# cloneofsimo/paint-with-words-sd

Measured on NVIDIA H100. Metric: unet_steps_per_sec_512sq_cfg, higher is better.
Workload: dtype f16

## Files before the change

### paint_with_words_sd_b200/csrc/pww_abi.cu

```cuda
#include <stdio.h>
#include <string.h>

#include "pww_common.cuh"
#include "xattn_tc.cuh"
#include "xattn_fused2.cuh"
#include "attn_tc.cuh"
#include "unet_ops.cuh"
#include "sampler_step.cuh"
#include "control_inject.cuh"
#include <stdlib.h>

namespace {

thread_local char g_last_cuda_error[640] = "";

int cuda_fail(cudaError_t e);

bool aligned16(const void* p) { return (reinterpret_cast<uintptr_t>(p) & 15u) == 0; }

bool supported_head_dim(int D) { return D == 40 || D == 64 || D == 80 || D == 160; }

int check_common(const void* q, const void* k, int B, int H, int N, int T, int D, int64_t q_bs, int64_t q_rs,
                 int64_t k_bs, int64_t k_rs) {
  if (!q || !k || B <= 0 || H <= 0 || N <= 0 || T <= 0 || D <= 0) return PWW_ERR_BAD_ARG;
  if (!aligned16(q) || !aligned16(k)) return PWW_ERR_BAD_ARG;
  if ((q_bs | q_rs | k_bs | k_rs) & 7) return PWW_ERR_BAD_ARG;
  if (q_rs < (int64_t)H * D || k_rs < (int64_t)H * D) return PWW_ERR_BAD_ARG;
  if (!supported_head_dim(D) || !pww::core::supported_keys(T)) return PWW_ERR_UNSUPPORTED;
  return PWW_OK;
}

template <int D_, int KC_>
struct Shape {
  static constexpr int D = D_, KC = KC_;
};
template <int D, typename F>
cudaError_t with_chunks(int T, F&& f) {
  switch (pww::core::chunks_of(T)) {
    case 1: return f(Shape<D, 1>{});
    case 2: return f(Shape<D, 2>{});
    case 3: return f(Shape<D, 3>{});
  }
  return cudaErrorInvalidValue;
}
template <typename F>
cudaError_t with_shape(int D, int T, F&& f) {
  switch (D) {
    case 40: return with_chunks<40>(T, f);
    case 64: return with_chunks<64>(T, f);
    case 80: return with_chunks<80>(T, f);
    case 160: return with_chunks<160>(T, f);
  }
  return cudaErrorInvalidValue;
}

size_t align_up(size_t x, size_t a) { return (x + a - 1) / a * a; }

int stats_slots_per_image(int, int) { return 2048; }

int cuda_fail(cudaError_t e) {
  snprintf(g_last_cuda_error, sizeof(g_last_cuda_error), "%s: %s %s", cudaGetErrorName(e), cudaGetErrorString(e),
           pww::tc::tc_error_buf());
  pww::tc::tc_error_buf()[0] = 0;
  return PWW_ERR_CUDA;
}

}

extern "C" {

int pww_version(void) { return 300; }

const char* pww_status_str(int status) {
  switch (status) {
    case PWW_OK: return "ok";
    case PWW_ERR_BAD_ARG: return "bad argument (null/misaligned pointer, non-positive size or stride not a multiple of 8)";
    case PWW_ERR_UNSUPPORTED: return "unsupported shape or dtype (head dim must be 40/64/80/160, T <= 80, 154 or 231)";
    case PWW_ERR_CUDA: return "CUDA error (see pww_last_cuda_error)";
    case PWW_ERR_WORKSPACE: return "workspace too small (see pww_xattn_workspace_bytes)";
    default: return "unknown status";
  }
}

const char* pww_last_cuda_error(void) { return g_last_cuda_error; }

int pww_device_supported(void) {
  int dev = 0, major = 0;
  cudaError_t e = cudaGetDevice(&dev);
  if (e != cudaSuccess) return cuda_fail(e);
  e = cudaDeviceGetAttribute(&major, cudaDevAttrComputeCapabilityMajor, dev);
  if (e != cudaSuccess) return cuda_fail(e);
  return major == 9 ? 1 : 0;
}

size_t pww_xattn_workspace_bytes(int B, int H, int N, int T, int D) {
  (void)T; (void)D;
  if (B <= 0 || H <= 0 || N <= 0) return 0;
  return align_up((size_t)B * sizeof(unsigned int), 256) +
         (size_t)B * stats_slots_per_image(H, N) * sizeof(pww::StatPartial);
}

}

namespace {

template <typename E>
int xattn_stats(const void* q, const void* k, int B, int H, int N, int T, int D, int64_t q_batch_stride,
                int64_t q_row_stride, int64_t k_batch_stride, int64_t k_row_stride, int stat, const int32_t* kinds,
                bool per_image, const int32_t* wmap_index, float* stats, void* workspace, size_t workspace_bytes,
                void* stream) {
  int rc = check_common(q, k, B, H, N, T, D, q_batch_stride, q_row_stride, k_batch_stride, k_row_stride);
  if (rc) return rc;
  if (!stats || !workspace) return PWW_ERR_BAD_ARG;
  if (per_image ? !kinds : (stat != PWW_STAT_MAX && stat != PWW_STAT_STD)) return PWW_ERR_BAD_ARG;
  if (workspace_bytes < pww_xattn_workspace_bytes(B, H, N, T, D)) return PWW_ERR_WORKSPACE;
  pww::XattnParams<E> p;
  memset(&p, 0, sizeof(p));
  p.q = (const E*)q; p.k = (const E*)k;
  p.B = B; p.H = H; p.N = N; p.T = T; p.D = D;
  p.q_bs = q_batch_stride; p.q_rs = q_row_stride; p.k_bs = k_batch_stride; p.k_rs = k_row_stride;
  p.wmap_index = wmap_index; p.stat = stat; p.stat_kind = per_image ? kinds : nullptr; p.stats_out = stats;
  p.counters = (unsigned int*)workspace;
  p.partials = (pww::StatPartial*)((char*)workspace + align_up((size_t)B * sizeof(unsigned int), 256));
  cudaStream_t s = (cudaStream_t)stream;
  {
    if (pww::tc::stats_slots() > stats_slots_per_image(H, N)) return PWW_ERR_WORKSPACE;
    for (int b0 = 0; b0 < B; b0 += pww::tc::kMaxBatch) {
      pww::XattnParams<E> c = p;
      c.B = (B - b0) < pww::tc::kMaxBatch ? (B - b0) : pww::tc::kMaxBatch;
      c.q = p.q + (int64_t)b0 * p.q_bs;
      c.k = p.k + (int64_t)b0 * p.k_bs;
      c.wmap_index = p.wmap_index ? p.wmap_index + b0 : nullptr;
      c.stat_kind = p.stat_kind ? p.stat_kind + b0 : nullptr;
      c.stats_out = p.stats_out + b0;
      const cudaError_t e = with_shape(D, T, [&](auto k) { return pww::tc::launch_stats<k.D, k.KC>(c, s); });
      if (e != cudaSuccess) return cuda_fail(e);
    }
    return PWW_OK;
  }
}

template <typename E>
int xattn_fwd(const void* q, const void* k, const void* v, void* out, int B, int H, int N, int T, int D,
              int64_t q_batch_stride, int64_t q_row_stride, int64_t k_batch_stride, int64_t k_row_stride,
              int64_t o_batch_stride, int64_t o_row_stride, const float* wmap, int64_t wmap_batch_stride,
              const int32_t* wmap_index, const float* stats, const float* g_sigma, int64_t g_stride, float scale,
              void* stream) {
  int rc = check_common(q, k, B, H, N, T, D, q_batch_stride, q_row_stride, k_batch_stride, k_row_stride);
  if (rc) return rc;
  if (!v || !out || !aligned16(v) || !aligned16(out)) return PWW_ERR_BAD_ARG;
  if ((o_batch_stride | o_row_stride) & 7 || o_row_stride < (int64_t)H * D) return PWW_ERR_BAD_ARG;
  if (wmap && (!stats || !g_sigma)) return PWW_ERR_BAD_ARG;
  pww::XattnParams<E> p;
  memset(&p, 0, sizeof(p));
  p.q = (const E*)q; p.k = (const E*)k; p.v = (const E*)v; p.out = (E*)out;
  p.B = B; p.H = H; p.N = N; p.T = T; p.D = D;
  p.q_bs = q_batch_stride; p.q_rs = q_row_stride; p.k_bs = k_batch_stride; p.k_rs = k_row_stride;
  p.o_bs = o_batch_stride; p.o_rs = o_row_stride;
  p.wmap = wmap; p.wmap_bs = wmap_batch_stride; p.wmap_index = wmap_index;
  p.stats = stats; p.g_sigma = g_sigma; p.g_stride = g_stride; p.scale = scale;
  cudaStream_t s = (cudaStream_t)stream;
  {
    for (int b0 = 0; b0 < B; b0 += pww::tc::kMaxBatch) {
      pww::XattnParams<E> c = p;
      c.B = (B - b0) < pww::tc::kMaxBatch ? (B - b0) : pww::tc::kMaxBatch;
      c.q = p.q + (int64_t)b0 * p.q_bs;
      c.k = p.k + (int64_t)b0 * p.k_bs;
      c.v = p.v + (int64_t)b0 * p.k_bs;
      c.out = p.out + (int64_t)b0 * p.o_bs;
      c.wmap_index = (p.wmap && p.wmap_index) ? p.wmap_index + b0 : nullptr;
      c.stats = p.stats ? p.stats + b0 : nullptr;
      c.g_sigma = p.g_sigma ? p.g_sigma + (int64_t)b0 * p.g_stride : nullptr;
      if (p.wmap && !p.wmap_index) c.wmap = p.wmap + (int64_t)b0 * p.wmap_bs;
      const cudaError_t e = with_shape(D, T, [&](auto k) { return pww::tc::launch_fwd<k.D, k.KC>(c, s); });
      if (e != cudaSuccess) return cuda_fail(e);
    }
    return PWW_OK;
  }
}

template <typename E>
int xattn_fused(const void* q, const void* k, const void* v, void* out, int B, int H, int N, int T, int D,
                int64_t q_batch_stride, int64_t q_row_stride, int64_t k_batch_stride, int64_t k_row_stride,
                int64_t o_batch_stride, int64_t o_row_stride, const void* mpack, int64_t mpack_batch_stride, int Bw,
                const int8_t* cidx, const int32_t* wmap_index, int stat, const int32_t* kinds, bool per_image,
                const float* g_sigma, float scale, float* stats, void* workspace, size_t workspace_bytes,
                void* stream) {
  int rc = check_common(q, k, B, H, N, T, D, q_batch_stride, q_row_stride, k_batch_stride, k_row_stride);
  if (rc) return rc;
  if (!v || !out || !aligned16(v) || !aligned16(out)) return PWW_ERR_BAD_ARG;
  if ((o_batch_stride | o_row_stride) & 7 || o_row_stride < (int64_t)H * D || o_batch_stride <= 0) return PWW_ERR_BAD_ARG;
  if (mpack) {
    if (!cidx || !g_sigma || !workspace || Bw <= 0 || !aligned16(mpack)) return PWW_ERR_BAD_ARG;
    if ((mpack_batch_stride & 7) || mpack_batch_stride < (int64_t)N * pww::fx::kMW) return PWW_ERR_BAD_ARG;
    if (per_image ? !kinds : (stat != PWW_STAT_MAX && stat != PWW_STAT_STD)) return PWW_ERR_BAD_ARG;
    if (workspace_bytes < pww_xattn_fused_workspace_bytes()) return PWW_ERR_WORKSPACE;
  }
  pww::XattnParams<E> p;
  memset(&p, 0, sizeof(p));
  p.q = (const E*)q; p.k = (const E*)k; p.v = (const E*)v; p.out = (E*)out;
  p.B = B; p.H = H; p.N = N; p.T = T; p.D = D;
  p.q_bs = q_batch_stride; p.q_rs = q_row_stride; p.k_bs = k_batch_stride; p.k_rs = k_row_stride;
  p.o_bs = o_batch_stride; p.o_rs = o_row_stride;
  p.g_sigma = g_sigma; p.g_stride = per_image ? 1 : 0; p.scale = scale; p.stat = stat;
  p.stat_kind = per_image ? kinds : nullptr;
  p.counters = (unsigned int*)workspace;
  p.partials = workspace ? (pww::StatPartial*)((char*)workspace + 512) : nullptr;
  cudaStream_t s = (cudaStream_t)stream;
  int chunk = pww::fx::kMaxBatch;
  {
    const int tiles = pww::ceil_div(N, pww::core::kBM);
    const int hg = pww::ceil_div(H, D == 40 ? pww::fx::Cfg2<40>::G : (D == 64 ? pww::fx::Cfg2<64>::G : 1));
    while (chunk > 1) {
      const int cb = B < chunk ? B : chunk;
      if (pww::fx::fused2_fits(cb, hg, tiles, pww::fx::fused_grid(cb * hg * tiles))) break;
      chunk >>= 1;
    }
  }
  for (int b0 = 0; b0 < B; b0 += chunk) {
    pww::XattnParams<E> c = p;
    c.B = (B - b0) < chunk ? (B - b0) : chunk;
    c.q = p.q + (int64_t)b0 * p.q_bs;
    c.k = p.k + (int64_t)b0 * p.k_bs;
    c.v = p.v + (int64_t)b0 * p.k_bs;
    c.out = p.out + (int64_t)b0 * p.o_bs;
    c.stats_out = stats ? stats + b0 : nullptr;
    c.stat_kind = p.stat_kind ? p.stat_kind + b0 : nullptr;
    c.g_sigma = p.g_sigma ? p.g_sigma + (int64_t)b0 * p.g_stride : nullptr;
    const void* mp = mpack;
    const int8_t* ci = cidx;
    if (mpack && wmap_index) {
      c.wmap_index = wmap_index + b0;
    } else if (mpack) {
      c.wmap_index = nullptr;
      mp = (const __half*)mpack + (int64_t)b0 * mpack_batch_stride;
      ci = cidx + (int64_t)b0 * pww::core::kTP * pww::core::chunks_of(T);
    }
    c.wmap = mpack ? (const float*)mp : nullptr;
    const cudaError_t e =
        with_shape(D, T, [&](auto k) { return pww::fx::launch_fused2<k.D, k.KC>(c, mp, mpack_batch_stride, ci, s); });
    if (e == cudaErrorInvalidConfiguration) return PWW_ERR_UNSUPPORTED;
    if (e != cudaSuccess) return cuda_fail(e);
  }
  return PWW_OK;
}

template <typename E>
int groupnorm_nhwc(const void* x, const void* add, int64_t add_batch_stride, const void* gamma, const void* beta, void* y,
                   int B, int HW, int C, int G, float eps, int silu, void* workspace, size_t workspace_bytes,
                   void* stream) {
  if (!x || !gamma || !beta || !y || !workspace || B <= 0 || HW <= 0 || C <= 0 || G <= 0) return PWW_ERR_BAD_ARG;
  if (!aligned16(x) || !aligned16(y) || !aligned16(gamma) || !aligned16(beta) || (add && !aligned16(add)))
    return PWW_ERR_BAD_ARG;
  if ((C & 7) || (C % G) || G > 64 || (C >> 3) > 1024) return PWW_ERR_UNSUPPORTED;
  if (add && ((add_batch_stride & 7) || add_batch_stride < C)) return PWW_ERR_BAD_ARG;
  if (workspace_bytes < pww_groupnorm_workspace_bytes(B, HW, G)) return PWW_ERR_WORKSPACE;
  pww::uops::GnParams<E> p;
  p.x = (const E*)x; p.add = (const E*)add; p.add_bs = add_batch_stride; p.gamma = (const E*)gamma; p.beta = (const E*)beta;
  p.y = (E*)y;
  char* w = (char*)workspace;
  p.counters = (unsigned int*)w;
  w += align_up((size_t)B * sizeof(unsigned int), 256);
  p.stats = (float*)w;
  w += align_up((size_t)B * G * 2 * sizeof(float), 256);
  p.partial = (float*)w;
  p.B = B; p.HW = HW; p.C = C; p.G = G; p.eps = eps; p.silu = silu;
  p.chunks = pww::uops::gn_chunks(HW);
  p.rows_per_chunk = (HW + p.chunks - 1) / p.chunks;
  cudaStream_t s = (cudaStream_t)stream;
  const int nvec = C >> 3;
  const int rpp = nvec >= 256 ? 1 : 256 / nvec;
  const size_t smem1 = (size_t)rpp * C * 2 * sizeof(float);
  if (smem1 > 48 * 1024) return PWW_ERR_UNSUPPORTED;
  pww::uops::gn_stats_kernel<E><<<dim3(p.chunks, B), nvec * rpp, smem1, s>>>(p);
  int rows_per_block = (int)(((long long)HW * B + 2 * pww::tc::num_sms() - 1) / (2 * pww::tc::num_sms()));
  if (rows_per_block < rpp) rows_per_block = rpp;
  if (rows_per_block > 32) rows_per_block = 32;
  pww::uops::gn_apply_kernel<E><<<dim3((HW + rows_per_block - 1) / rows_per_block, B), nvec * rpp, 0, s>>>(p, rows_per_block);
  cudaError_t e = cudaGetLastError();
  return e == cudaSuccess ? PWW_OK : cuda_fail(e);
}

template <typename E>
int geglu(const void* in, void* out, int64_t M, int I, void* stream) {
  if (!in || !out || M <= 0 || I <= 0 || !aligned16(in) || !aligned16(out)) return PWW_ERR_BAD_ARG;
  if (I & 7) return PWW_ERR_UNSUPPORTED;
  const long long total = (long long)M * (I >> 3);
  long long blocks = (total + 255) / 256;
  const long long cap = (long long)pww::tc::num_sms() * 16;
  if (blocks > cap) blocks = cap;
  pww::uops::geglu_kernel<E><<<(int)blocks, 256, 0, (cudaStream_t)stream>>>((const E*)in, (E*)out, M, I);
  cudaError_t e = cudaGetLastError();
  return e == cudaSuccess ? PWW_OK : cuda_fail(e);
}

template <typename E>
int add_layernorm(const void* x, const void* res, const void* gamma, const void* beta, void* sum_out, void* y, int64_t M,
                  int C, float eps, void* stream) {
  if (!x || !gamma || !beta || !y || M <= 0 || C <= 0) return PWW_ERR_BAD_ARG;
  if (!aligned16(x) || !aligned16(y) || !aligned16(gamma) || !aligned16(beta) || (res && !aligned16(res)) ||
      (sum_out && !aligned16(sum_out)))
    return PWW_ERR_BAD_ARG;
  if ((C & 7) || C > 2048) return PWW_ERR_UNSUPPORTED;
  const int vpl = ((C >> 3) + 31) / 32;
  const int warps = 8;
  const unsigned grid = (unsigned)((M + warps - 1) / warps);
  cudaStream_t s = (cudaStream_t)stream;
  const E *xp = (const E*)x, *rp = (const E*)res, *gp = (const E*)gamma, *bp = (const E*)beta;
  E *sp = (E*)sum_out, *yp = (E*)y;
  switch (vpl) {
    case 1: pww::uops::add_layernorm_kernel<E, 1><<<grid, warps * 32, 0, s>>>(xp, rp, gp, bp, sp, yp, M, C, eps); break;
    case 2: pww::uops::add_layernorm_kernel<E, 2><<<grid, warps * 32, 0, s>>>(xp, rp, gp, bp, sp, yp, M, C, eps); break;
    case 3: pww::uops::add_layernorm_kernel<E, 3><<<grid, warps * 32, 0, s>>>(xp, rp, gp, bp, sp, yp, M, C, eps); break;
    case 4: pww::uops::add_layernorm_kernel<E, 4><<<grid, warps * 32, 0, s>>>(xp, rp, gp, bp, sp, yp, M, C, eps); break;
    case 5: pww::uops::add_layernorm_kernel<E, 5><<<grid, warps * 32, 0, s>>>(xp, rp, gp, bp, sp, yp, M, C, eps); break;
    case 6: pww::uops::add_layernorm_kernel<E, 6><<<grid, warps * 32, 0, s>>>(xp, rp, gp, bp, sp, yp, M, C, eps); break;
    case 7: pww::uops::add_layernorm_kernel<E, 7><<<grid, warps * 32, 0, s>>>(xp, rp, gp, bp, sp, yp, M, C, eps); break;
    case 8: pww::uops::add_layernorm_kernel<E, 8><<<grid, warps * 32, 0, s>>>(xp, rp, gp, bp, sp, yp, M, C, eps); break;
    default: return PWW_ERR_UNSUPPORTED;
  }
  cudaError_t e = cudaGetLastError();
  return e == cudaSuccess ? PWW_OK : cuda_fail(e);
}

template <typename E>
int attn_fwd(const void* q, const void* k, const void* v, void* out, int B, int H, int N, int D, int64_t qkv_batch_stride,
             int64_t qkv_row_stride, int64_t o_batch_stride, int64_t o_row_stride, float scale, void* stream) {
  if (!q || !k || !v || !out || B <= 0 || H <= 0 || N <= 0 || D <= 0) return PWW_ERR_BAD_ARG;
  if (!aligned16(q) || !aligned16(k) || !aligned16(v) || !aligned16(out)) return PWW_ERR_BAD_ARG;
  if ((qkv_batch_stride | qkv_row_stride | o_batch_stride | o_row_stride) & 7) return PWW_ERR_BAD_ARG;
  if (qkv_row_stride < (int64_t)H * D || o_row_stride < (int64_t)H * D) return PWW_ERR_BAD_ARG;
  if (!supported_head_dim(D)) return PWW_ERR_UNSUPPORTED;
  cudaStream_t s = (cudaStream_t)stream;
  cudaError_t e = cudaErrorInvalidValue;
  const int64_t bs = qkv_batch_stride, rs = qkv_row_stride, obs = o_batch_stride, ors = o_row_stride;
  switch (D) {
    case 40: e = pww::fa::launch<40, E>(q, k, v, out, B, H, N, bs, rs, obs, ors, scale, s); break;
    case 64: e = pww::fa::launch<64, E>(q, k, v, out, B, H, N, bs, rs, obs, ors, scale, s); break;
    case 80: e = pww::fa::launch<80, E>(q, k, v, out, B, H, N, bs, rs, obs, ors, scale, s); break;
    case 160: e = pww::fa::launch<160, E>(q, k, v, out, B, H, N, bs, rs, obs, ors, scale, s); break;
  }
  return e == cudaSuccess ? PWW_OK : cuda_fail(e);
}

template <typename E>
int control_inject(int n, void* const* dst, const void* const* res, const int64_t* elems_per_image, int rows,
                   const float* scales, void* stream) {
  if (n < 1 || n > pww::ctl::kMaxLevels || rows < 1 || !dst || !res || !elems_per_image) return PWW_ERR_BAD_ARG;
  pww::ctl::InjectArgs a;
  a.off[0] = 0;
  for (int k = 0; k < n; ++k) {
    const int64_t e = elems_per_image[k];
    if (e <= 0 || (e % pww::ctl::kVec) != 0) return PWW_ERR_BAD_ARG;
    if (!dst[k] || !res[k] || !aligned16(dst[k]) || !aligned16(res[k])) return PWW_ERR_BAD_ARG;
    a.dst[k] = dst[k];
    a.res[k] = res[k];
    a.vec_per_image[k] = e / pww::ctl::kVec;
    a.off[k + 1] = a.off[k] + (int64_t)rows * a.vec_per_image[k];
  }
  for (int k = n; k < pww::ctl::kMaxLevels; ++k) {
    a.dst[k] = nullptr;
    a.res[k] = nullptr;
    a.vec_per_image[k] = 0;
    a.off[k + 1] = a.off[n];
  }
  a.scales = scales;
  a.n = n;
  a.rows = rows;
  const cudaError_t e = pww::ctl::launch_inject<E>(a, (int64_t)pww::tc::num_sms() * 8, (cudaStream_t)stream);
  return e == cudaSuccess ? PWW_OK : cuda_fail(e);
}

}

extern "C" {

int pww_xattn_stats_f16(const void* q, const void* k, int B, int H, int N, int T, int D, int64_t q_batch_stride,
    int64_t q_row_stride, int64_t k_batch_stride, int64_t k_row_stride, int stat, const int32_t* wmap_index,
    float* stats, void* workspace, size_t workspace_bytes, void* stream) {
  return xattn_stats<__half>(
      q, k, B, H, N, T, D, q_batch_stride, q_row_stride, k_batch_stride, k_row_stride, stat, nullptr, false,
      wmap_index, stats, workspace, workspace_bytes, stream);
}
int pww_xattn_stats_bf16(const void* q, const void* k, int B, int H, int N, int T, int D, int64_t q_batch_stride,
    int64_t q_row_stride, int64_t k_batch_stride, int64_t k_row_stride, int stat, const int32_t* wmap_index,
    float* stats, void* workspace, size_t workspace_bytes, void* stream) {
  return xattn_stats<__nv_bfloat16>(
      q, k, B, H, N, T, D, q_batch_stride, q_row_stride, k_batch_stride, k_row_stride, stat, nullptr, false,
      wmap_index, stats, workspace, workspace_bytes, stream);
}

int pww_xattn_stats_multi_f16(const void* q, const void* k, int B, int H, int N, int T, int D, int64_t q_batch_stride,
    int64_t q_row_stride, int64_t k_batch_stride, int64_t k_row_stride, const int32_t* stat, const int32_t* wmap_index,
    float* stats, void* workspace, size_t workspace_bytes, void* stream) {
  return xattn_stats<__half>(
      q, k, B, H, N, T, D, q_batch_stride, q_row_stride, k_batch_stride, k_row_stride, PWW_STAT_MAX, stat, true,
      wmap_index, stats, workspace, workspace_bytes, stream);
}
int pww_xattn_stats_multi_bf16(const void* q, const void* k, int B, int H, int N, int T, int D, int64_t q_batch_stride,
    int64_t q_row_stride, int64_t k_batch_stride, int64_t k_row_stride, const int32_t* stat, const int32_t* wmap_index,
    float* stats, void* workspace, size_t workspace_bytes, void* stream) {
  return xattn_stats<__nv_bfloat16>(
      q, k, B, H, N, T, D, q_batch_stride, q_row_stride, k_batch_stride, k_row_stride, PWW_STAT_MAX, stat, true,
      wmap_index, stats, workspace, workspace_bytes, stream);
}

int pww_xattn_fwd_f16(const void* q, const void* k, const void* v, void* out, int B, int H, int N, int T, int D,
    int64_t q_batch_stride, int64_t q_row_stride, int64_t k_batch_stride, int64_t k_row_stride, int64_t o_batch_stride,
    int64_t o_row_stride, const float* wmap, int64_t wmap_batch_stride, const int32_t* wmap_index, const float* stats,
    const float* g_sigma, float scale, void* stream) {
  return xattn_fwd<__half>(q, k, v, out, B, H, N, T, D, q_batch_stride, q_row_stride, k_batch_stride, k_row_stride,
      o_batch_stride, o_row_stride, wmap, wmap_batch_stride, wmap_index, stats, g_sigma, 0, scale, stream);
}
int pww_xattn_fwd_bf16(const void* q, const void* k, const void* v, void* out, int B, int H, int N, int T, int D,
    int64_t q_batch_stride, int64_t q_row_stride, int64_t k_batch_stride, int64_t k_row_stride, int64_t o_batch_stride,
    int64_t o_row_stride, const float* wmap, int64_t wmap_batch_stride, const int32_t* wmap_index, const float* stats,
    const float* g_sigma, float scale, void* stream) {
  return xattn_fwd<__nv_bfloat16>(
      q, k, v, out, B, H, N, T, D, q_batch_stride, q_row_stride, k_batch_stride, k_row_stride,
      o_batch_stride, o_row_stride, wmap, wmap_batch_stride, wmap_index, stats, g_sigma, 0, scale, stream);
}

int pww_xattn_fwd_multi_f16(const void* q, const void* k, const void* v, void* out, int B, int H, int N, int T, int D,
    int64_t q_batch_stride, int64_t q_row_stride, int64_t k_batch_stride, int64_t k_row_stride, int64_t o_batch_stride,
    int64_t o_row_stride, const float* wmap, int64_t wmap_batch_stride, const int32_t* wmap_index, const float* stats,
    const float* g_sigma, float scale, void* stream) {
  return xattn_fwd<__half>(q, k, v, out, B, H, N, T, D, q_batch_stride, q_row_stride, k_batch_stride, k_row_stride,
      o_batch_stride, o_row_stride, wmap, wmap_batch_stride, wmap_index, stats, g_sigma, 1, scale, stream);
}
int pww_xattn_fwd_multi_bf16(const void* q, const void* k, const void* v, void* out, int B, int H, int N, int T, int D,
    int64_t q_batch_stride, int64_t q_row_stride, int64_t k_batch_stride, int64_t k_row_stride, int64_t o_batch_stride,
    int64_t o_row_stride, const float* wmap, int64_t wmap_batch_stride, const int32_t* wmap_index, const float* stats,
    const float* g_sigma, float scale, void* stream) {
  return xattn_fwd<__nv_bfloat16>(
      q, k, v, out, B, H, N, T, D, q_batch_stride, q_row_stride, k_batch_stride, k_row_stride,
      o_batch_stride, o_row_stride, wmap, wmap_batch_stride, wmap_index, stats, g_sigma, 1, scale, stream);
}

size_t pww_xattn_fused_workspace_bytes(void) { return pww::fx::fused_workspace_bytes(); }

int pww_xattn_fused_f16(const void* q, const void* k, const void* v, void* out, int B, int H, int N, int T, int D,
    int64_t q_batch_stride, int64_t q_row_stride, int64_t k_batch_stride, int64_t k_row_stride, int64_t o_batch_stride,
    int64_t o_row_stride, const void* mpack, int64_t mpack_batch_stride, int Bw, const int8_t* cidx,
    const int32_t* wmap_index, int stat, const float* g_sigma, float scale, float* stats, void* workspace,
    size_t workspace_bytes, void* stream) {
  return xattn_fused<__half>(q, k, v, out, B, H, N, T, D, q_batch_stride, q_row_stride, k_batch_stride, k_row_stride,
      o_batch_stride, o_row_stride, mpack, mpack_batch_stride, Bw, cidx, wmap_index, stat, nullptr, false,
      g_sigma, scale, stats, workspace, workspace_bytes, stream);
}
int pww_xattn_fused_bf16(const void* q, const void* k, const void* v, void* out, int B, int H, int N, int T, int D,
    int64_t q_batch_stride, int64_t q_row_stride, int64_t k_batch_stride, int64_t k_row_stride, int64_t o_batch_stride,
    int64_t o_row_stride, const void* mpack, int64_t mpack_batch_stride, int Bw, const int8_t* cidx,
    const int32_t* wmap_index, int stat, const float* g_sigma, float scale, float* stats, void* workspace,
    size_t workspace_bytes, void* stream) {
  return xattn_fused<__nv_bfloat16>(
      q, k, v, out, B, H, N, T, D, q_batch_stride, q_row_stride, k_batch_stride, k_row_stride,
      o_batch_stride, o_row_stride, mpack, mpack_batch_stride, Bw, cidx, wmap_index, stat, nullptr, false,
      g_sigma, scale, stats, workspace, workspace_bytes, stream);
}

int pww_xattn_fused_multi_f16(const void* q, const void* k, const void* v, void* out, int B, int H, int N, int T, int D,
    int64_t q_batch_stride, int64_t q_row_stride, int64_t k_batch_stride, int64_t k_row_stride, int64_t o_batch_stride,
    int64_t o_row_stride, const void* mpack, int64_t mpack_batch_stride, int Bw, const int8_t* cidx,
    const int32_t* wmap_index, const int32_t* stat, const float* g_sigma, float scale, float* stats, void* workspace,
    size_t workspace_bytes, void* stream) {
  return xattn_fused<__half>(q, k, v, out, B, H, N, T, D, q_batch_stride, q_row_stride, k_batch_stride, k_row_stride,
      o_batch_stride, o_row_stride, mpack, mpack_batch_stride, Bw, cidx, wmap_index, PWW_STAT_MAX, stat, true,
      g_sigma, scale, stats, workspace, workspace_bytes, stream);
}
int pww_xattn_fused_multi_bf16(const void* q, const void* k, const void* v, void* out, int B, int H, int N, int T, int D,
    int64_t q_batch_stride, int64_t q_row_stride, int64_t k_batch_stride, int64_t k_row_stride, int64_t o_batch_stride,
    int64_t o_row_stride, const void* mpack, int64_t mpack_batch_stride, int Bw, const int8_t* cidx,
    const int32_t* wmap_index, const int32_t* stat, const float* g_sigma, float scale, float* stats, void* workspace,
    size_t workspace_bytes, void* stream) {
  return xattn_fused<__nv_bfloat16>(
      q, k, v, out, B, H, N, T, D, q_batch_stride, q_row_stride, k_batch_stride, k_row_stride,
      o_batch_stride, o_row_stride, mpack, mpack_batch_stride, Bw, cidx, wmap_index, PWW_STAT_MAX, stat, true,
      g_sigma, scale, stats, workspace, workspace_bytes, stream);
}

int pww_attn_fwd_f16(const void* q, const void* k, const void* v, void* out, int B, int H, int N, int D,
    int64_t qkv_batch_stride, int64_t qkv_row_stride, int64_t o_batch_stride, int64_t o_row_stride, float scale,
    void* stream) {
  return attn_fwd<__half>(
      q, k, v, out, B, H, N, D, qkv_batch_stride, qkv_row_stride, o_batch_stride, o_row_stride, scale, stream);
}
int pww_attn_fwd_bf16(const void* q, const void* k, const void* v, void* out, int B, int H, int N, int D,
    int64_t qkv_batch_stride, int64_t qkv_row_stride, int64_t o_batch_stride, int64_t o_row_stride, float scale,
    void* stream) {
  return attn_fwd<__nv_bfloat16>(
      q, k, v, out, B, H, N, D, qkv_batch_stride, qkv_row_stride, o_batch_stride, o_row_stride, scale, stream);
}

size_t pww_groupnorm_workspace_bytes(int B, int HW, int G) {
  if (B <= 0 || HW <= 0 || G <= 0) return 0;
  return align_up((size_t)B * sizeof(unsigned int), 256) + align_up((size_t)B * G * 2 * sizeof(float), 256) +
         (size_t)B * pww::uops::gn_chunks(HW) * G * 2 * sizeof(float);
}

int pww_groupnorm_nhwc_f16(const void* x, const void* add, int64_t add_batch_stride, const void* gamma,
    const void* beta, void* y, int B, int HW, int C, int G, float eps, int silu, void* workspace, size_t workspace_bytes,
    void* stream) {
  return groupnorm_nhwc<__half>(
      x, add, add_batch_stride, gamma, beta, y, B, HW, C, G, eps, silu, workspace, workspace_bytes,
      stream);
}
int pww_groupnorm_nhwc_bf16(const void* x, const void* add, int64_t add_batch_stride, const void* gamma,
    const void* beta, void* y, int B, int HW, int C, int G, float eps, int silu, void* workspace, size_t workspace_bytes,
    void* stream) {
  return groupnorm_nhwc<__nv_bfloat16>(
      x, add, add_batch_stride, gamma, beta, y, B, HW, C, G, eps, silu, workspace, workspace_bytes,
      stream);
}

int pww_geglu_f16(const void* in, void* out, int64_t M, int I, void* stream) {
  return geglu<__half>(in, out, M, I, stream);
}
int pww_geglu_bf16(const void* in, void* out, int64_t M, int I, void* stream) {
  return geglu<__nv_bfloat16>(in, out, M, I, stream);
}

int pww_add_layernorm_f16(const void* x, const void* res, const void* gamma, const void* beta, void* sum_out, void* y,
    int64_t M, int C, float eps, void* stream) {
  return add_layernorm<__half>(x, res, gamma, beta, sum_out, y, M, C, eps, stream);
}
int pww_add_layernorm_bf16(const void* x, const void* res, const void* gamma, const void* beta, void* sum_out, void* y,
    int64_t M, int C, float eps, void* stream) {
  return add_layernorm<__nv_bfloat16>(x, res, gamma, beta, sum_out, y, M, C, eps, stream);
}

int pww_sampler_input(const float* latents, const float* scale, const float* extra, void* out, int out_dtype, int m,
                      int channels, int height, int width, void* stream) {
  if (!latents || !scale || !out || m <= 0 || height <= 0 || width <= 0) return PWW_ERR_BAD_ARG;
  if (channels != 4 && channels != 9) return PWW_ERR_BAD_ARG;
  if ((channels == 9) != (extra != nullptr)) return PWW_ERR_BAD_ARG;
  if (out_dtype != PWW_DTYPE_F32 && out_dtype != PWW_DTYPE_F16 && out_dtype != PWW_DTYPE_BF16) return PWW_ERR_UNSUPPORTED;
  pww::smp::InputArgs a;
  a.lat = latents; a.scale = scale; a.extra = extra; a.out = out; a.m = m; a.C = channels; a.hw = height * width;
  const bool px4 = (a.hw % 4) == 0 && aligned16(latents) && (!extra || aligned16(extra)) && aligned16(out);
  cudaStream_t s = (cudaStream_t)stream;
  const cudaError_t e = out_dtype == PWW_DTYPE_F16    ? pww::smp::launch_input<__half>(a, px4, s)
                        : out_dtype == PWW_DTYPE_BF16 ? pww::smp::launch_input<__nv_bfloat16>(a, px4, s)
                                                      : pww::smp::launch_input<float>(a, px4, s);
  return e == cudaSuccess ? PWW_OK : cuda_fail(e);
}

int pww_sampler_update(const void* eps, int eps_dtype, int64_t eps_batch_stride, int64_t eps_channel_stride,
                       int64_t eps_row_stride, int64_t eps_col_stride, float* latents, float* history, int history_len,
                       const float* noise, const float* guidance, const float* beta, const float* form, int m,
                       int height, int width, void* stream) {
  if (!eps || !latents || !history || !guidance || !beta || !form) return PWW_ERR_BAD_ARG;
  if (m <= 0 || height <= 0 || width <= 0 || history_len < 1 || history_len > 4) return PWW_ERR_BAD_ARG;
  if (eps_dtype != PWW_DTYPE_F32 && eps_dtype != PWW_DTYPE_F16 && eps_dtype != PWW_DTYPE_BF16) return PWW_ERR_UNSUPPORTED;
  pww::smp::UpdateArgs a;
  a.eps = eps; a.e_sn = eps_batch_stride; a.e_sc = eps_channel_stride; a.e_sh = eps_row_stride; a.e_sw = eps_col_stride;
  a.lat = latents; a.hist = history; a.noise = noise; a.gscale = guidance; a.beta = beta; a.form = form;
  a.m = m; a.h = height; a.w = width; a.nh = history_len;
  const int64_t hw = (int64_t)height * width;
  const size_t es = eps_dtype == PWW_DTYPE_F32 ? 4 : 2;
  const bool px4 = (hw % 4) == 0 && aligned16(latents) && aligned16(history) && (!noise || aligned16(noise));
  const size_t need = px4 ? 16 : 4 * es;
  const bool cl = eps_channel_stride == 1 && eps_col_stride == 4 && eps_row_stride == 4 * (int64_t)width &&
                  (reinterpret_cast<uintptr_t>(eps) % need) == 0 && ((size_t)eps_batch_stride * es) % need == 0;
  cudaStream_t s = (cudaStream_t)stream;
  const cudaError_t e = eps_dtype == PWW_DTYPE_F16    ? pww::smp::launch_update<__half>(a, px4, cl, s)
                        : eps_dtype == PWW_DTYPE_BF16 ? pww::smp::launch_update<__nv_bfloat16>(a, px4, cl, s)
                                                      : pww::smp::launch_update<float>(a, px4, cl, s);
  return e == cudaSuccess ? PWW_OK : cuda_fail(e);
}

int pww_control_inject_f16(int n, void* const* dst, const void* const* res, const int64_t* elems_per_image, int rows,
                           const float* scales, void* stream) {
  return control_inject<__half>(n, dst, res, elems_per_image, rows, scales, stream);
}
int pww_control_inject_bf16(int n, void* const* dst, const void* const* res, const int64_t* elems_per_image, int rows,
                            const float* scales, void* stream) {
  return control_inject<__nv_bfloat16>(n, dst, res, elems_per_image, rows, scales, stream);
}

int pww_debug_fwd_schedule(int B, int H, int tiles, int grid, const int* wmap_index, int* out) {
  if (!wmap_index || !out) return PWW_ERR_BAD_ARG;
  return pww::tc::fwd_schedule_host(B, H, tiles, grid, wmap_index, out);
}

int pww_debug_set_fused_grid(int grid) {
  pww::fx::debug_grid() = grid < 0 ? 0 : grid;
  return PWW_OK;
}
int pww_debug_fused2_schedule(int B, int H, int G, int tiles, int grid, const int* wmap_index, int* out, int max_jobs) {
  if (!wmap_index || !out) return PWW_ERR_BAD_ARG;
  return pww::fx::fused2_schedule_host(B, H, G, tiles, grid, wmap_index, out, max_jobs);
}
int pww_debug_fused2_heads_per_unit(void) { return pww::fx::Cfg2<40>::G; }
int pww_debug_set_fused_jobs_dump(void* device_buffer) {
  pww::fx::debug_jobs_dump() = (unsigned*)device_buffer;
  return PWW_OK;
}
int pww_debug_fused_cta_has_image(int cta, int grid, int B, int H, int tiles, const int* wmap_index, int b) {
  if (!wmap_index) return PWW_ERR_BAD_ARG;
  return pww::fx::fused_cta_has_image_host(cta, grid, B, H, tiles, wmap_index, b);
}

}
```

Measured before the change: 129.9.

## Add Hopper wgmma flash-attention kernel for head-dim 40 self-attention

```diff
diff --git a/paint_with_words_sd_b200/csrc/attn_wgmma.cuh b/paint_with_words_sd_b200/csrc/attn_wgmma.cuh
--- /dev/null
+++ b/paint_with_words_sd_b200/csrc/attn_wgmma.cuh
@@ -0,0 +1,177 @@
+#pragma once
+#include "attn_tc.cuh"
+#include "mma_sm90.cuh"
+#include "pww_common.cuh"
+#include "wgmma_sm90.cuh"
+#include "xattn_core.cuh"
+#include "xattn_tc.cuh"
+
+namespace pww {
+namespace fa3 {
+
+constexpr int kBM = 128;
+constexpr int kThreads = 256;
+
+template <int D>
+struct Cfg {
+  static_assert(D == 40, "head dim served by the warpgroup-MMA kernel (wgmma_sm90.cuh has its N = 40 and 64 forms)");
+  static constexpr int DP = (D + 15) / 16 * 16;
+  static constexpr int KS = DP / 16;
+  static constexpr int NT = D / 8;
+  static constexpr int BN = 64;
+  static constexpr int STAGES = 3;
+  static constexpr uint32_t RG = DP * 16;
+  static constexpr uint32_t QBYTES = kBM * DP * 2;
+  static constexpr uint32_t TBYTES = BN * DP * 2;
+  static constexpr uint32_t SMEM = QBYTES + STAGES * 2 * TBYTES;
+  static_assert(2 * (SMEM + 1024) <= 233472, "two CTAs per SM");
+  static_assert(8 * 16 * core::Tile<D>::LD * 2 <= SMEM, "output staging of core::warp_store fits");
+};
+
+template <int D, int R, typename E>
+__device__ __forceinline__ void load_tile(uint32_t dst, const E* src, int64_t rs, int valid) {
+  using CF = Cfg<D>;
+  constexpr int CH = CF::DP / 8, DCH = D / 8;
+#pragma unroll
+  for (int idx = threadIdx.x; idx < R * CH; idx += kThreads) {
+    const int rl = idx & 7, c = (idx >> 3) % CH, rg = (idx >> 3) / CH;
+    const int r = rg * 8 + rl;
+    const bool ok = r < valid && c < DCH;
+    ptx::cp_async16(dst + rg * CF::RG + c * 128 + rl * 16, ok ? (const void*)(src + (int64_t)r * rs + c * 8) : (const void*)src,
+                    ok ? 16u : 0u);
+  }
+}
+
+template <int D, typename E>
+__global__ void __launch_bounds__(kThreads, 2) attn_wgmma_kernel(const fa::Params<E> p) {
+  using CF = Cfg<D>;
+  constexpr int BN = CF::BN;
+  extern __shared__ __align__(128) unsigned char smem[];
+  const uint32_t s0 = ptx::smem_u32(smem);
+  const int warp = threadIdx.x >> 5, lane = threadIdx.x & 31, wg = warp >> 2;
+  const int qtiles = (p.N + kBM - 1) / kBM;
+  const int bh = blockIdx.x / qtiles, qt = blockIdx.x - bh * qtiles;
+  const int b = bh / p.H, h = bh - b * p.H;
+  const int row_base = qt * kBM;
+  const E* qb = p.q + (int64_t)b * p.bs + h * D;
+  const E* kb = p.k + (int64_t)b * p.bs + h * D;
+  const E* vb = p.v + (int64_t)b * p.bs + h * D;
+  const int ntiles = (p.N + BN - 1) / BN;
+  auto stage = [&](int j) { return s0 + CF::QBYTES + (uint32_t)(j % CF::STAGES) * 2u * CF::TBYTES; };
+  auto issue_kv = [&](int j) {
+    if (j < ntiles) {
+      const int rows = p.N - j * BN < BN ? p.N - j * BN : BN;
+      load_tile<D, BN>(stage(j), kb + (int64_t)j * BN * p.rs, p.rs, rows);
+      load_tile<D, BN>(stage(j) + CF::TBYTES, vb + (int64_t)j * BN * p.rs, p.rs, rows);
+    }
+    ptx::cp_async_commit();
+  };
+  load_tile<D, kBM>(s0, qb + (int64_t)row_base * p.rs, p.rs, p.N - row_base < kBM ? p.N - row_base : kBM);
+#pragma unroll
+  for (int j = 0; j < CF::STAGES - 1; ++j) issue_kv(j);
+
+  float o[CF::NT][4];
+  float(&of)[D / 2] = reinterpret_cast<float(&)[D / 2]>(o);
+#pragma unroll
+  for (int i = 0; i < D / 2; ++i) of[i] = 0.f;
+  float m0 = -INFINITY, m1 = -INFINITY, l0 = 0.f, l1 = 0.f;
+  const float sl2 = p.scale * 1.4426950408889634f;
+  const uint64_t dq = ptx::wgmma_desc(s0 + (uint32_t)wg * 8u * CF::RG, 128, CF::RG);
+#pragma unroll 1
+  for (int jt = 0; jt < ntiles; ++jt) {
+    ptx::cp_async_wait<CF::STAGES - 2>();
+    ptx::fence_proxy_async_smem();
+    __syncthreads();
+    issue_kv(jt + CF::STAGES - 1);
+    const uint32_t ks = stage(jt), vs = ks + CF::TBYTES;
+    float s[BN / 2];
+    ptx::wgmma_fence();
+    ptx::wgmma_ss_first<E>(s, dq, ptx::wgmma_desc(ks, 128, CF::RG));
+#pragma unroll
+    for (int kk = 1; kk < CF::KS; ++kk)
+      ptx::wgmma_ss<E>(s, dq + (uint64_t)(kk * 16), ptx::wgmma_desc(ks + kk * 256, 128, CF::RG), 1);
+    ptx::wgmma_commit();
+    ptx::wgmma_wait<0>();
+    ptx::reg_fence(s);
+    const int valid = p.N - jt * BN;
+    if (valid < BN) {
+#pragma unroll
+      for (int j = 0; j < BN / 8; ++j)
+#pragma unroll
+        for (int e = 0; e < 4; ++e)
+          if (core::tok(j, e, lane) >= valid) s[4 * j + e] = -INFINITY;
+    }
+    float t0 = -INFINITY, t1 = -INFINITY;
+#pragma unroll
+    for (int j = 0; j < BN / 8; ++j) {
+      t0 = fmaxf(t0, fmaxf(s[4 * j], s[4 * j + 1]));
+      t1 = fmaxf(t1, fmaxf(s[4 * j + 2], s[4 * j + 3]));
+    }
+    t0 = fmaxf(t0, __shfl_xor_sync(0xffffffffu, t0, 1));
+    t0 = fmaxf(t0, __shfl_xor_sync(0xffffffffu, t0, 2));
+    t1 = fmaxf(t1, __shfl_xor_sync(0xffffffffu, t1, 1));
+    t1 = fmaxf(t1, __shfl_xor_sync(0xffffffffu, t1, 2));
+    const float mn0 = fmaxf(m0, t0), mn1 = fmaxf(m1, t1);
+    const float a0 = ptx::ex2((m0 - mn0) * sl2), a1 = ptx::ex2((m1 - mn1) * sl2);
+    m0 = mn0; m1 = mn1;
+    const float n0 = -mn0 * sl2, n1 = -mn1 * sl2;
+    uint32_t pa[BN / 16][4];
+    float r0 = 0.f, r1 = 0.f;
+#pragma unroll
+    for (int j = 0; j < BN / 8; ++j) {
+      const float p0 = ptx::ex2(fmaf(s[4 * j], sl2, n0)), p1 = ptx::ex2(fmaf(s[4 * j + 1], sl2, n0));
+      const float p2 = ptx::ex2(fmaf(s[4 * j + 2], sl2, n1)), p3 = ptx::ex2(fmaf(s[4 * j + 3], sl2, n1));
+      r0 += p0 + p1;
+      r1 += p2 + p3;
+      pa[j >> 1][(j & 1) * 2] = ptx::pack2<E>(p0, p1);
+      pa[j >> 1][(j & 1) * 2 + 1] = ptx::pack2<E>(p2, p3);
+    }
+    l0 = l0 * a0 + r0;
+    l1 = l1 * a1 + r1;
+#pragma unroll
+    for (int j = 0; j < CF::NT; ++j) {
+      o[j][0] *= a0; o[j][1] *= a0; o[j][2] *= a1; o[j][3] *= a1;
+    }
+    ptx::reg_fence(of);
+    ptx::wgmma_fence();
+#pragma unroll
+    for (int kk = 0; kk < BN / 16; ++kk) ptx::wgmma_rs<E>(of, pa[kk], ptx::wgmma_desc(vs + kk * 2 * CF::RG, CF::RG, 128), 1);
+    ptx::wgmma_commit();
+    ptx::wgmma_wait<0>();
+    ptx::reg_fence(of);
+  }
+  l0 += __shfl_xor_sync(0xffffffffu, l0, 1);
+  l0 += __shfl_xor_sync(0xffffffffu, l0, 2);
+  l1 += __shfl_xor_sync(0xffffffffu, l1, 1);
+  l1 += __shfl_xor_sync(0xffffffffu, l1, 2);
+  const float i0 = 1.f / l0, i1 = 1.f / l1;
+#pragma unroll
+  for (int j = 0; j < CF::NT; ++j) {
+    o[j][0] *= i0; o[j][1] *= i0; o[j][2] *= i1; o[j][3] *= i1;
+  }
+  __syncthreads();
+  core::warp_store<D>(o, smem + warp * 16 * core::Tile<D>::LD * 2, lane, p.out + (int64_t)b * p.o_bs + h * D, p.o_rs,
+                      row_base + warp * 16, p.N);
+}
+
+template <int D, typename E>
+cudaError_t launch(const void* q, const void* k, const void* v, void* out, int B, int H, int N, int64_t bs, int64_t rs,
+                   int64_t o_bs, int64_t o_rs, float scale, cudaStream_t s) {
+  using CF = Cfg<D>;
+  fa::Params<E> p;
+  p.q = (const E*)q; p.k = (const E*)k; p.v = (const E*)v; p.out = (E*)out;
+  p.B = B; p.H = H; p.N = N; p.bs = bs; p.rs = rs; p.o_bs = o_bs; p.o_rs = o_rs; p.scale = scale;
+  static bool attr_set[tc::kMaxDevices] = {false};
+  if (!attr_set[tc::cur_device()]) {
+    cudaError_t e = cudaFuncSetAttribute(attn_wgmma_kernel<D, E>, cudaFuncAttributeMaxDynamicSharedMemorySize, CF::SMEM);
+    if (e != cudaSuccess) return e;
+    attr_set[tc::cur_device()] = true;
+  }
+  const long long grid = (long long)B * H * ((N + kBM - 1) / kBM);
+  if (grid > 0x7fffffffLL) return cudaErrorInvalidConfiguration;
+  attn_wgmma_kernel<D, E><<<(unsigned)grid, kThreads, CF::SMEM, s>>>(p);
+  return cudaGetLastError();
+}
+
+}
+}
diff --git a/paint_with_words_sd_b200/csrc/pww_abi.cu b/paint_with_words_sd_b200/csrc/pww_abi.cu
--- a/paint_with_words_sd_b200/csrc/pww_abi.cu
+++ b/paint_with_words_sd_b200/csrc/pww_abi.cu
@@ -5,6 +5,7 @@
 #include "xattn_tc.cuh"
 #include "xattn_fused2.cuh"
 #include "attn_tc.cuh"
+#include "attn_wgmma.cuh"
 #include "unet_ops.cuh"
 #include "sampler_step.cuh"
 #include "control_inject.cuh"
@@ -323,6 +324,8 @@
   return e == cudaSuccess ? PWW_OK : cuda_fail(e);
 }
 
+constexpr int kSelfAttnWgmmaMinKeys = 1024;
+
 template <typename E>
 int attn_fwd(const void* q, const void* k, const void* v, void* out, int B, int H, int N, int D, int64_t qkv_batch_stride,
              int64_t qkv_row_stride, int64_t o_batch_stride, int64_t o_row_stride, float scale, void* stream) {
@@ -335,7 +338,10 @@
   cudaError_t e = cudaErrorInvalidValue;
   const int64_t bs = qkv_batch_stride, rs = qkv_row_stride, obs = o_batch_stride, ors = o_row_stride;
   switch (D) {
-    case 40: e = pww::fa::launch<40, E>(q, k, v, out, B, H, N, bs, rs, obs, ors, scale, s); break;
+    case 40:
+      e = N > kSelfAttnWgmmaMinKeys ? pww::fa3::launch<40, E>(q, k, v, out, B, H, N, bs, rs, obs, ors, scale, s)
+                                    : pww::fa::launch<40, E>(q, k, v, out, B, H, N, bs, rs, obs, ors, scale, s);
+      break;
     case 64: e = pww::fa::launch<64, E>(q, k, v, out, B, H, N, bs, rs, obs, ors, scale, s); break;
     case 80: e = pww::fa::launch<80, E>(q, k, v, out, B, H, N, bs, rs, obs, ors, scale, s); break;
     case 160: e = pww::fa::launch<160, E>(q, k, v, out, B, H, N, bs, rs, obs, ors, scale, s); break;
diff --git a/paint_with_words_sd_b200/csrc/wgmma_sm90.cuh b/paint_with_words_sd_b200/csrc/wgmma_sm90.cuh
--- /dev/null
+++ b/paint_with_words_sd_b200/csrc/wgmma_sm90.cuh
@@ -0,0 +1,91 @@
+#pragma once
+#include <cuda_runtime.h>
+#include <stdint.h>
+
+#include <type_traits>
+
+#include "pww_common.cuh"
+
+namespace pww {
+namespace ptx {
+
+__device__ __forceinline__ uint64_t wgmma_desc(uint32_t addr, uint32_t lbo, uint32_t sbo) {
+  return (uint64_t)((addr & 0x3FFFFu) >> 4) | ((uint64_t)(lbo >> 4) << 16) | ((uint64_t)(sbo >> 4) << 32);
+}
+
+__device__ __forceinline__ void wgmma_fence() { asm volatile("wgmma.fence.sync.aligned;" ::: "memory"); }
+__device__ __forceinline__ void wgmma_commit() { asm volatile("wgmma.commit_group.sync.aligned;" ::: "memory"); }
+template <int N>
+__device__ __forceinline__ void wgmma_wait() { asm volatile("wgmma.wait_group.sync.aligned %0;" ::"n"(N) : "memory"); }
+template <int R>
+__device__ __forceinline__ void reg_fence(float (&d)[R]) {
+#pragma unroll
+  for (int i = 0; i < R; ++i) asm volatile("" : "+f"(d[i])::"memory");
+}
+__device__ __forceinline__ void fence_proxy_async_smem() { asm volatile("fence.proxy.async.shared::cta;" ::: "memory"); }
+
+template <typename E>
+__device__ __forceinline__ void wgmma_ss(float (&d)[32], uint64_t da, uint64_t db, int scale_d) {
+  if constexpr (std::is_same_v<E, __half>) {
+    asm volatile(
+        "{\n.reg .pred p;\nsetp.ne.b32 p, %34, 0;\n"
+        "wgmma.mma_async.sync.aligned.m64n64k16.f32.f16.f16 "
+        "{%0, %1, %2, %3, %4, %5, %6, %7, %8, %9, %10, %11, %12, %13, %14, %15, %16, %17, %18, %19, %20, %21, %22, %23, %24, %25, %26, %27, %28, %29, %30, %31}, "
+        "%32, %33, p, 1, 1, 0, 0;\n}\n"
+        : "+f"(d[0]), "+f"(d[1]), "+f"(d[2]), "+f"(d[3]), "+f"(d[4]), "+f"(d[5]), "+f"(d[6]), "+f"(d[7]), "+f"(d[8]), "+f"(d[9]), "+f"(d[10]), "+f"(d[11]), "+f"(d[12]), "+f"(d[13]), "+f"(d[14]), "+f"(d[15]), "+f"(d[16]), "+f"(d[17]), "+f"(d[18]), "+f"(d[19]), "+f"(d[20]), "+f"(d[21]), "+f"(d[22]), "+f"(d[23]), "+f"(d[24]), "+f"(d[25]), "+f"(d[26]), "+f"(d[27]), "+f"(d[28]), "+f"(d[29]), "+f"(d[30]), "+f"(d[31])
+        : "l"(da), "l"(db), "r"(scale_d));
+  } else {
+    asm volatile(
+        "{\n.reg .pred p;\nsetp.ne.b32 p, %34, 0;\n"
+        "wgmma.mma_async.sync.aligned.m64n64k16.f32.bf16.bf16 "
+        "{%0, %1, %2, %3, %4, %5, %6, %7, %8, %9, %10, %11, %12, %13, %14, %15, %16, %17, %18, %19, %20, %21, %22, %23, %24, %25, %26, %27, %28, %29, %30, %31}, "
+        "%32, %33, p, 1, 1, 0, 0;\n}\n"
+        : "+f"(d[0]), "+f"(d[1]), "+f"(d[2]), "+f"(d[3]), "+f"(d[4]), "+f"(d[5]), "+f"(d[6]), "+f"(d[7]), "+f"(d[8]), "+f"(d[9]), "+f"(d[10]), "+f"(d[11]), "+f"(d[12]), "+f"(d[13]), "+f"(d[14]), "+f"(d[15]), "+f"(d[16]), "+f"(d[17]), "+f"(d[18]), "+f"(d[19]), "+f"(d[20]), "+f"(d[21]), "+f"(d[22]), "+f"(d[23]), "+f"(d[24]), "+f"(d[25]), "+f"(d[26]), "+f"(d[27]), "+f"(d[28]), "+f"(d[29]), "+f"(d[30]), "+f"(d[31])
+        : "l"(da), "l"(db), "r"(scale_d));
+  }
+}
+
+template <typename E>
+__device__ __forceinline__ void wgmma_ss_first(float (&d)[32], uint64_t da, uint64_t db) {
+  if constexpr (std::is_same_v<E, __half>) {
+    asm volatile(
+        "{\n.reg .pred p;\nsetp.ne.b32 p, 0, 0;\n"
+        "wgmma.mma_async.sync.aligned.m64n64k16.f32.f16.f16 "
+        "{%0, %1, %2, %3, %4, %5, %6, %7, %8, %9, %10, %11, %12, %13, %14, %15, %16, %17, %18, %19, %20, %21, %22, %23, %24, %25, %26, %27, %28, %29, %30, %31}, "
+        "%32, %33, p, 1, 1, 0, 0;\n}\n"
+        : "=f"(d[0]), "=f"(d[1]), "=f"(d[2]), "=f"(d[3]), "=f"(d[4]), "=f"(d[5]), "=f"(d[6]), "=f"(d[7]), "=f"(d[8]), "=f"(d[9]), "=f"(d[10]), "=f"(d[11]), "=f"(d[12]), "=f"(d[13]), "=f"(d[14]), "=f"(d[15]), "=f"(d[16]), "=f"(d[17]), "=f"(d[18]), "=f"(d[19]), "=f"(d[20]), "=f"(d[21]), "=f"(d[22]), "=f"(d[23]), "=f"(d[24]), "=f"(d[25]), "=f"(d[26]), "=f"(d[27]), "=f"(d[28]), "=f"(d[29]), "=f"(d[30]), "=f"(d[31])
+        : "l"(da), "l"(db));
+  } else {
+    asm volatile(
+        "{\n.reg .pred p;\nsetp.ne.b32 p, 0, 0;\n"
+        "wgmma.mma_async.sync.aligned.m64n64k16.f32.bf16.bf16 "
+        "{%0, %1, %2, %3, %4, %5, %6, %7, %8, %9, %10, %11, %12, %13, %14, %15, %16, %17, %18, %19, %20, %21, %22, %23, %24, %25, %26, %27, %28, %29, %30, %31}, "
+        "%32, %33, p, 1, 1, 0, 0;\n}\n"
+        : "=f"(d[0]), "=f"(d[1]), "=f"(d[2]), "=f"(d[3]), "=f"(d[4]), "=f"(d[5]), "=f"(d[6]), "=f"(d[7]), "=f"(d[8]), "=f"(d[9]), "=f"(d[10]), "=f"(d[11]), "=f"(d[12]), "=f"(d[13]), "=f"(d[14]), "=f"(d[15]), "=f"(d[16]), "=f"(d[17]), "=f"(d[18]), "=f"(d[19]), "=f"(d[20]), "=f"(d[21]), "=f"(d[22]), "=f"(d[23]), "=f"(d[24]), "=f"(d[25]), "=f"(d[26]), "=f"(d[27]), "=f"(d[28]), "=f"(d[29]), "=f"(d[30]), "=f"(d[31])
+        : "l"(da), "l"(db));
+  }
+}
+
+template <typename E>
+__device__ __forceinline__ void wgmma_rs(float (&d)[20], const uint32_t (&a)[4], uint64_t db, int scale_d) {
+  if constexpr (std::is_same_v<E, __half>) {
+    asm volatile(
+        "{\n.reg .pred p;\nsetp.ne.b32 p, %25, 0;\n"
+        "wgmma.mma_async.sync.aligned.m64n40k16.f32.f16.f16 "
+        "{%0, %1, %2, %3, %4, %5, %6, %7, %8, %9, %10, %11, %12, %13, %14, %15, %16, %17, %18, %19}, "
+        "{%20, %21, %22, %23}, %24, p, 1, 1, 1;\n}\n"
+        : "+f"(d[0]), "+f"(d[1]), "+f"(d[2]), "+f"(d[3]), "+f"(d[4]), "+f"(d[5]), "+f"(d[6]), "+f"(d[7]), "+f"(d[8]), "+f"(d[9]), "+f"(d[10]), "+f"(d[11]), "+f"(d[12]), "+f"(d[13]), "+f"(d[14]), "+f"(d[15]), "+f"(d[16]), "+f"(d[17]), "+f"(d[18]), "+f"(d[19])
+        : "r"(a[0]), "r"(a[1]), "r"(a[2]), "r"(a[3]), "l"(db), "r"(scale_d));
+  } else {
+    asm volatile(
+        "{\n.reg .pred p;\nsetp.ne.b32 p, %25, 0;\n"
+        "wgmma.mma_async.sync.aligned.m64n40k16.f32.bf16.bf16 "
+        "{%0, %1, %2, %3, %4, %5, %6, %7, %8, %9, %10, %11, %12, %13, %14, %15, %16, %17, %18, %19}, "
+        "{%20, %21, %22, %23}, %24, p, 1, 1, 1;\n}\n"
+        : "+f"(d[0]), "+f"(d[1]), "+f"(d[2]), "+f"(d[3]), "+f"(d[4]), "+f"(d[5]), "+f"(d[6]), "+f"(d[7]), "+f"(d[8]), "+f"(d[9]), "+f"(d[10]), "+f"(d[11]), "+f"(d[12]), "+f"(d[13]), "+f"(d[14]), "+f"(d[15]), "+f"(d[16]), "+f"(d[17]), "+f"(d[18]), "+f"(d[19])
+        : "r"(a[0]), "r"(a[1]), "r"(a[2]), "r"(a[3]), "l"(db), "r"(scale_d));
+  }
+}
+
+}
+}
```

Result: no change. 130.6, median of 6 (+0.5%).
